# ActiveIntelligentSystemsLab/moving_object_detector

Measured on AMD Instinct MI355X. Metric: stereo pairs/sec (scene-flow+cluster) at 1280x720, higher is better.
Workload: dtype f32+f64; 1 GPU; 1280x720 synthetic sequence (zed-style camera), scene-flow + cluster kernels only (disparity/flow precomputed, HBM-resident), reference default parameters; distinct_frames_per_gpu=16, outputs=six cloud planes, dynamic mask, objects, cluster-label plane, batch_chunks=0, stream=one synthetic stream, contiguous chunk per rank + one disparity plane of halo, collective_executed=True, collective_backend=nccl, collective_on_device=True, collective_world_size=1

## Files before the change

moving_object_detector_amd/csrc/ccl_bits.hip:

```cpp
#include "cluster_common.h"
#pragma clang fp contract(off)
namespace {

namespace bits {
constexpr int TH = 16;

struct Row3 { uint32_t h, a, b; };

__device__ __forceinline__ Row3 operator|(Row3 x, Row3 y) { return {x.h | y.h, x.a | y.a, x.b | y.b}; }
__device__ __forceinline__ Row3 operator&(Row3 x, Row3 y) { return {x.h & y.h, x.a & y.a, x.b & y.b}; }
__device__ __forceinline__ Row3 operator^(Row3 x, Row3 y) { return {x.h ^ y.h, x.a ^ y.a, x.b ^ y.b}; }
__device__ __forceinline__ Row3 andn(Row3 x, Row3 y) { return {x.h & ~y.h, x.a & ~y.a, x.b & ~y.b}; }
__device__ __forceinline__ bool any(Row3 x) { return (x.h | x.a | x.b) != 0u; }
template <int K> __device__ __forceinline__ Row3 shl(Row3 v) {
  return {v.h << K, __builtin_amdgcn_alignbit(v.a, v.h, 32 - K), __builtin_amdgcn_alignbit(v.b, v.a, 32 - K)};
}
template <int K, int NH> __device__ __forceinline__ Row3 shr(Row3 v) {
  return {__builtin_amdgcn_alignbit(v.a, v.h, K) & (~0u << (32 - NH)), __builtin_amdgcn_alignbit(v.b, v.a, K), v.b >> K};
}
__device__ __forceinline__ uint32_t dn1(uint32_t v) { return (uint32_t)__builtin_amdgcn_update_dpp(0, (int)v, 0x138, 0xF, 0xF, false); }
__device__ __forceinline__ uint32_t up1(uint32_t v) { return (uint32_t)__builtin_amdgcn_update_dpp(0, (int)v, 0x130, 0xF, 0xF, false); }
__device__ __forceinline__ Row3 row_dn(Row3 v) { return {dn1(v.h), dn1(v.a), dn1(v.b)}; }
__device__ __forceinline__ Row3 row_up(Row3 v) { return {up1(v.h), up1(v.a), up1(v.b)}; }
template <int K, bool DN> __device__ __forceinline__ Row3 row_shift(Row3 v) {
// ... 54 lines not shown
  return __builtin_amdgcn_readlane(v, 0) + __builtin_amdgcn_readlane(v, 16);
}
__device__ __forceinline__ uint64_t lane_bits(uint32_t lo, uint32_t hi, int l) {
  return ((uint64_t)(uint32_t)__builtin_amdgcn_readlane((int)hi, l) << 32) | (uint64_t)(uint32_t)__builtin_amdgcn_readlane((int)lo, l);
}

constexpr int kTilesPerBlock = 1, kMaxClasses = 4, kMaxComps = 32;

template <class T> __device__ __forceinline__ T ldo(const void *base, uint32_t byte_off) { return *(const T *)((const char *)base + byte_off); }
template <class T> __device__ __forceinline__ void sto(void *base, uint32_t byte_off, T v) { *(T *)((char *)base + byte_off) = v; }

template <int HL>
__global__ __launch_bounds__(64 * kTilesPerBlock) void k_ccl_bits(DevCam c, ClArgs a, int tiles_x, int tiles_y) {
  constexpr int PH = TH + HL;
  const int lane = threadIdx.x, wv = __builtin_amdgcn_readfirstlane((int)threadIdx.y);
  const int wi = blockIdx.x * kTilesPerBlock + wv, ty = blockIdx.y, f = blockIdx.z;
  if (wi >= tiles_x) return;
  const size_t tix = (size_t)f * tiles_y * tiles_x + (size_t)ty * tiles_x + wi;
  int *hdr = a.tilehdr + tix * 2;
  if (__builtin_amdgcn_readfirstlane(hdr[0]) == 0) return;
  const int x0 = wi * 64, y0 = ty * TH, MW = c.mask_words, W = c.W, H = c.H;
  const size_t N = (size_t)W * H, fN = (size_t)f * N;
  Row3 Mrem;
  {
    const int gy = y0 - HL + lane;
    const bool inrow = lane < PH && gy >= 0 && gy < H;
    const uint64_t *mr = a.mask + ((size_t)f * H + (inrow ? gy : 0)) * MW;
    const uint64_t q0 = mr[wi], qL = mr[max(wi - 1, 0)];
    Mrem.h = (inrow && wi > 0) ? ((uint32_t)(qL >> 32) & (~0u << (32 - HL))) : 0u;
    Mrem.a = inrow ? (uint32_t)q0 : 0u;
    Mrem.b = inrow ? (uint32_t)(q0 >> 32) : 0u;
  }
  const bool il = lane >= HL && lane < PH;
  const float th = c.depth_th, qnan = __uint_as_float(0x7fc00000u);
  const uint32_t oc = 4u * (uint32_t)min(x0 + lane, W - 1);
  uint32_t rootA = 0u, rootB = 0u;
  int nreq = 0, ncomp = 0;
  uint2 *req = a.requests + tix * a.req_cap;
  float hi_prev = 0.0f;
  bool bail = false;
  const float *zplane = a.z + fN;
  __shared__ float zlds[kTilesPerBlock][PH][64];
  float(*zl)[64] = zlds[wv];
  float zh[HL];
  float lo = qnan, hi = qnan;
  bool need_z = true;
  if (a.zrange) {
    const int gy = y0 - HL + lane;
    const bool inrow = lane < PH && gy >= 0 && gy < H;
    const float2 *zr = a.zrange + ((size_t)f * H + (inrow ? gy : 0)) * MW;
    const float2 r0 = zr[wi], rL = zr[max(wi - 1, 0)];
    const bool u0 = (Mrem.a | Mrem.b) != 0u, uL = Mrem.h != 0u;
    lo = zmin(u0 ? r0.x : qnan, uL ? rL.x : qnan); hi = zmax(u0 ? r0.y : qnan, uL ? rL.y : qnan);
    lo = wave_fmin(lo); hi = wave_fmax(hi);
    need_z = hi - lo > th;
  }
  if (need_z) {
    lo = qnan; hi = qnan;
    {
      const int gy = min(max(y0 - HL + lane, 0), H - 1);
      const int hx = max(x0 - HL, 0);
#pragma unroll
      for (int j = 0; j < HL; j++) zh[j] = ldo<float>(zplane, 4u * (uint32_t)(gy * W + min(hx + j, W - 1)));
    }
    uint64_t nanb = 0ull;
    constexpr int HB = (PH + 1) / 2;
// ... 90 lines not shown
    const uint64_t ne = __ballot(any(M));
    const int first = __builtin_ctzll(ne);
    const Row3 starts = andn(C, shl<1>(C));
    const bool ok = !any(M) || (popc3(starts) == 1 && !any(E ^ M) && (lane == first || any(M & above)));
    single = __ballot(!ok) == 0ull && __ballot(any(R)) != 0ull;
  }
  for (;;) {
    const uint64_t rrows = __ballot(any(R));
    if (rrows == 0ull) break;
    Row3 S;
    if (single) S = M;
    else {
      const int sr = __builtin_ctzll(rrows);
      const uint32_t sa = (uint32_t)__builtin_amdgcn_readlane((int)R.a, sr), sb = (uint32_t)__builtin_amdgcn_readlane((int)R.b, sr);
      const uint32_t ba = sa & (0u - sa), bb = sa ? 0u : (sb & (0u - sb));
      S = {0u, lane == sr ? ba : 0u, lane == sr ? bb : 0u};
      for (;;) {
        Row3 rA, rX, lA, lX;
        dil_r<HL>(S, rA, rX);
        dil_l<HL>(S, lA, lX);
        const Row3 reach = M & (rA | lA | vert<HL, true>(rA) | vert<HL, false>(lA));
        const Row3 S2 = (fill_up(C, reach) | rev(fill_up(rC, rev(reach)))) & M;
        const bool grew = any(S2 ^ S);
        S = S2;
        if (__ballot(grew) == 0ull) break;
      }
    }
    const uint64_t irows = __ballot(il && (S.a | S.b) != 0u);
    const int rr = __builtin_ctzll(irows);
    const uint32_t fa = (uint32_t)__builtin_amdgcn_readlane((int)S.a, rr), fb = (uint32_t)__builtin_amdgcn_readlane((int)S.b, rr);
    const int rcol = fa ? __builtin_ctz(fa) : 32 + __builtin_ctz(fb);
    const int rootg = (y0 + rr - HL) * W + x0 + rcol;
    if (lane == rr) { if (rcol < 32) rootA |= 1u << rcol; else rootB |= 1u << (rcol - 32); }
    int *pplane = a.parent + fN;
    uint32_t po = 4u * (uint32_t)(y0 * W + x0 + lane);
    asm volatile("" : "+v"(po));
#pragma unroll
    for (int j = 0; j < TH; j++) {
      const uint64_t bitsj = lane_bits(S.a, S.b, HL + j);
      if (bitsj != 0ull && __builtin_amdgcn_inverse_ballot_w64(bitsj))
        sto<int>(pplane, po + 4u * (uint32_t)(j * W), rootg);
    }
    {
      const int cnt = il ? __popc(S.a) + __popc(S.b) : 0;
      const uint32_t ka = S.a & UL.a, kb = S.b & UL.b;
      uint32_t key = (uint32_t)kKeyNone;
      if (il && (ka | kb)) key = (uint32_t)((y0 + lane - HL) * W + x0 + (ka ? __builtin_ctz(ka) : 32 + __builtin_ctz(kb)));
      const int size = wave_sum_lo32(cnt);
      key = wave_min_u32(key);
      if (lane == 0) { sto<int>(a.rsize + fN, 4u * (uint32_t)rootg, size); sto<int>(a.rkey + fN, 4u * (uint32_t)rootg, (int)key); }
    }
    {
      const Row3 HS = {S.h, lane < HL ? S.a : 0u, lane < HL ? S.b : 0u};
      const Row3 em = andn(HS, shl<1>(HS) | row_dn(HS));
      uint64_t todo = __ballot(any(em));
      while (todo) {
        const int l = __builtin_ctzll(todo);
        todo &= todo - 1ull;
        const uint64_t eb = lane_bits(em.a, em.b, l);
        const uint32_t eh = (uint32_t)__builtin_amdgcn_readlane((int)em.h, l) >> (32 - HL);
        const int hgrow = (y0 - HL + l) * W + x0;
        if (__builtin_amdgcn_inverse_ballot_w64((uint64_t)eh)) {
          const int slot = nreq + __popc(eh & ((1u << lane) - 1u));
          if (MOD_CHECK(a, slot < a.req_cap, 12)) req[slot] = make_uint2((uint32_t)(hgrow - HL + lane), (uint32_t)rootg);
        }
        nreq += __popc(eh);
        if (eb != 0ull && __builtin_amdgcn_inverse_ballot_w64(eb)) {
          const int slot = nreq + __popcll((unsigned long long)(eb & ((1ull << lane) - 1ull)));
          if (MOD_CHECK(a, slot < a.req_cap, 12)) req[slot] = make_uint2((uint32_t)(hgrow + lane), (uint32_t)rootg);
        }
        nreq += __popcll((unsigned long long)eb);
      }
    }
    if (single) break;
    R = andn(R, S);
    if (++ncomp >= kMaxComps && __ballot(any(R)) != 0ull) { bail = true; break; }
  }
  {
    uint64_t todo = __ballot((Za | Zb) != 0u);
    while (todo) {
      const int l = __builtin_ctzll(todo);
      todo &= todo - 1ull;
      if (__builtin_amdgcn_inverse_ballot_w64(lane_bits(Za, Zb, l))) {
        const int p = (y0 + l - HL) * W + x0 + lane;
        sto<int>(a.parent + fN, 4u * (uint32_t)p, p); sto<int>(a.rsize + fN, 4u * (uint32_t)p, 1); sto<int>(a.rkey + fN, 4u * (uint32_t)p, kKeyNone);
      }
    }
  }
    if (bail || __ballot(any(Mrem)) == 0ull) break;
  }
  if (bail) {
    if (lane == 0) a.tilelist[atomicAdd(&a.counters[4], 1)] = (uint32_t)tix;
    return;
  }
  if (il && y0 + lane - HL < H) a.lroot[((size_t)f * H + (y0 + lane - HL)) * MW + wi] = ((uint64_t)rootB << 32) | rootA;
  if (lane == 0) { hdr[1] = nreq; hdr[0] = 2; }
}
}
}

void launch_ccl_bits(const DevCam &c, const ClArgs &a, int frames, hipStream_t s) {
  const dim3 tgrid = tile_grid(c, frames);
  const int tx = (int)tgrid.x, tyn = (int)tgrid.y;
  const dim3 bgrid((tgrid.x + bits::kTilesPerBlock - 1) / bits::kTilesPerBlock, tgrid.y, tgrid.z), bblock(64, bits::kTilesPerBlock, 1);
  switch (c.n) {
#define MOD_BITS_CASE(n) case n: hipLaunchKernelGGL(bits::k_ccl_bits<n>, bgrid, bblock, 0, s, c, a, tx, tyn); break;
    MOD_BITS_CASE(1) MOD_BITS_CASE(2) MOD_BITS_CASE(3) MOD_BITS_CASE(4) MOD_BITS_CASE(5)
    MOD_BITS_CASE(6) MOD_BITS_CASE(7) MOD_BITS_CASE(8) MOD_BITS_CASE(9) MOD_BITS_CASE(10)
#undef MOD_BITS_CASE
  }
}
```

moving_object_detector_amd/csrc/ccl_merge.hip:

```cpp
#include "cluster_common.h"
#pragma clang fp contract(off)
namespace {

template <int TH>
__global__ __launch_bounds__(256) void k_tile_flags(DevCam c, ClArgs a, int tiles_x, int tiles_per_frame, int total) {
  const int t = blockIdx.x * 256 + threadIdx.x;
  if (t >= total) return;
  const int f = t / tiles_per_frame, tt = t - f * tiles_per_frame, ty = tt / tiles_x, wi = tt - ty * tiles_x;
  const uint64_t *m = a.mask + ((size_t)f * c.H + (size_t)ty * TH) * c.mask_words + wi;
  const int rows = min(TH, c.H - ty * TH);
  uint64_t any = 0;
#pragma unroll 4
  for (int r = 0; r < rows; r++) any |= m[(size_t)r * c.mask_words];
  a.tilehdr[(size_t)t * 2] = any != 0 ? 1 : 0;
  a.tilehdr[(size_t)t * 2 + 1] = 0;
}

constexpr int kLinkTiles = 32;

__global__ __launch_bounds__(256) void k_ccl_link(DevCam c, ClArgs a, int tiles_per_frame) {
  const int f = blockIdx.y, tid = threadIdx.x, lane = tid & 63;
  const int t0 = blockIdx.x * kLinkTiles;
  int cnt[kLinkTiles], total = 0;
#pragma unroll
  for (int u = 0; u < kLinkTiles; u++) {
    cnt[u] = 0;
    if (t0 + u < tiles_per_frame) {
      const int *hdr = a.tilehdr + ((size_t)f * tiles_per_frame + t0 + u) * 2;
      cnt[u] = hdr[0] ? hdr[1] : 0;
    }
    total += cnt[u];
  }
  if (total == 0) return;
  const size_t N = (size_t)c.W * c.H;
  int *parent = a.parent + (size_t)f * N;
  for (int i0 = 0; i0 < total; i0 += 256) {
    int i = i0 + tid, u = 0;
#pragma unroll
    for (int v = 0; v < kLinkTiles - 1; v++) if (u == v && i >= cnt[v]) { i -= cnt[v]; u = v + 1; }
    int ra = -1, rb = -1;
    if (i0 + tid < total) {
      const uint2 q = a.requests[((size_t)f * tiles_per_frame + t0 + u) * a.req_cap + i];
      if (MOD_CHECK(a, (size_t)q.x < N && (size_t)q.y < N, 0)) { ra = parent[q.x]; rb = (int)q.y; }
      if (!MOD_CHECK(a, ra < 0 || ((size_t)ra < N && rb >= 0), 1)) ra = -1;
    }
    const int pa = wave_prev_i32(ra), pb = wave_prev_i32(rb);
    if (ra >= 0 && !(lane > 0 && pa == ra && pb == rb)) uf_unite(parent, ra, rb);
  }
}

__device__ void select_frame(const DevCam &c, const ClArgs &a, ClusterInfo *tmp, int f, int tid);

template <int TH, bool FILTER>
__global__ __launch_bounds__(256) void k_ccl_merge(DevCam c, ClArgs a, int tiles_per_frame, ClusterInfo *tmp) {
  static_assert(64 % TH == 0, "a wave covers whole tiles");
  constexpr int TPW = 64 / TH;
  const int f = blockIdx.y, lane = threadIdx.x & 63, wv = threadIdx.x >> 6;
  const int t = (blockIdx.x * 4 + wv) * TPW + lane / TH, j = lane % TH;
  const size_t N = (size_t)c.W * c.H;
  int *parent = a.parent + (size_t)f * N;
  int *rsize = a.rsize + (size_t)f * N, *rkey = a.rkey + (size_t)f * N;
  const int wi = t % c.mask_words, ty = t / c.mask_words, y = ty * TH + j;
  unsigned long long bits = 0ull;
  if (t < tiles_per_frame && y < c.H && a.tilehdr[((size_t)f * tiles_per_frame + t) * 2] != 0)
    bits = a.lroot[((size_t)f * c.H + y) * c.mask_words + wi];
  while (bits) {
    const int b = __ffsll(bits) - 1;
    bits &= bits - 1ull;
    const int p = y * c.W + wi * 64 + b;
    const int r = uf_find(parent, p);
    if (!MOD_CHECK(a, r >= 0 && (size_t)r < N, 2)) continue;
    if (r == p) {
      const int slot = atomicAdd(&a.counters[f * 8 + 0], 1);
      if (MOD_CHECK(a, slot >= 0 && (size_t)slot < N, 3)) st_agent(&a.rootlist[(size_t)f * N + slot], p);
    } else {
      parent[p] = r;
// ... 96 lines not shown
```

moving_object_detector_amd/csrc/ccl_tile.hip:

```cpp
#include "cluster_common.h"
#include <algorithm>
#pragma clang fp contract(off)
namespace {

__device__ __forceinline__ void wave_accumulate(int *sizes, int *keys, int stride, int rec_idx, uint32_t key, int lane) {
  uint64_t todo = __ballot(rec_idx >= 0);
  while (todo) {
    const int leader = __ffsll((unsigned long long)todo) - 1;
    const int lid = __builtin_amdgcn_readlane(rec_idx, leader);
    const bool mine = rec_idx == lid;
    const uint64_t grp = __ballot(mine);
    const uint32_t k = wave_min_u32(mine ? key : (uint32_t)kKeyNone);
    if (lane == leader) {
      atomicAdd(&sizes[(size_t)lid * stride], __popcll((unsigned long long)grp));
      if (k != (uint32_t)kKeyNone) atomicMin(&keys[(size_t)lid * stride], (int)k);
    }
    todo &= ~grp;
  }
}

constexpr int kHaloBit = 0x8000;
__device__ __forceinline__ int lds_find(int *L, int a) {
  int p = ld_relaxed(L + (a & 0x7fff));
  while (p != a) {
// ... 292 lines not shown
      float zq[NMAX + 1];
#pragma unroll
      for (int k = 0; k <= NMAX; k++) zq[k] = zt[base - k];
      uint32_t gmask = 0;
#pragma unroll
      for (int k = 0; k <= NMAX; k++) gmask |= (fabsf(zp - zq[k]) > th) ? 0u : (1u << k);
      const uint32_t vmask = cand & gmask;
      const bool need_any = (vmask & dmask) != 0;
      up = up || (vmask != 0);
      if (!MOD_ABLATE(c, 1) && __ballot(need_any)) {
        COUNT(10, 1)
#pragma unroll
        for (int k = 0; k <= NMAX; k++) {
          if (k > n || (dv == 0 && k == 0)) continue;
          const int lab = lq[k];
          const bool need = ((vmask >> k) & 1u) && lab != cur && lab != last;
          if (__ballot(need)) {
            COUNT(12, 1)
            const int pl = wave_prev_i32(lab), pc = wave_prev_i32(cur), pn = wave_prev_i32((int)need);
            push_jobs(need && !(lane > 0 && pn && pc == cur && pl == lab), cur, lab);
            if (need) last = lab;
          }
        }
      }
    }
    STAMP(3)
    upr[j] = up;
  }
  run_jobs();
  lds_barrier();
  STAMP(4)
  int rootg[RPW], rootc[RPW];
  uint64_t rootbits[RPW];
#pragma unroll
  for (int j = 0; j < RPW; j++) {
    const int rr = w + NW * j, gy = y0 + rr;
    const bool dyn = (m0[rr + NMAX] >> lane) & 1ull;
    int rg = -1, rc = -1;
    bool isroot = false;
    if (dyn) {
      const int me = (rr + NMAX) * PW + NMAX + lane;
      const int r = lds_find(Lt, me);
      const int rgr = r / PW, rgc = r - rgr * PW;
      rg = (y0 + rgr - NMAX) * c.W + x0 + rgc - NMAX;
      rc = r;
      if (MOD_CHECK(a, rg >= 0 && (size_t)rg < N && rgr >= NMAX && rgc >= NMAX, 13)) a.parent[fN + (size_t)gy * c.W + x0 + lane] = rg;
      isroot = (r == me);
    }
    rootg[j] = rg; rootc[j] = rc;
    const uint64_t rb = __ballot(isroot);
    rootbits[j] = rb;
    if (lane == 0 && gy < c.H) a.lroot[((size_t)f * c.H + gy) * MW + wi] = rb;
  }
  STAMP(5)
  if (MOD_ABLATE(c, 1 << 18)) return;
  {
    const int topcells = n * (64 + n);
    const int total = topcells + TH * n;
    auto cell_of = [&](int i, int &gr, int &gc) {
      if (i < topcells) { gr = NMAX - n + i / (64 + n); gc = NMAX - n + i % (64 + n); }
      else { const int t = i - topcells; gr = NMAX + t / n; gc = NMAX - n + t % n; }
    };
    auto halo_dyn = [&](int gr, int gc) {
      const int gx = x0 - NMAX + gc;
      const uint64_t mw = (gc >= NMAX) ? m0[gr] : mL[gr];
      return gx >= 0 && ((mw >> (gx & 63)) & 1ull);
    };
    const bool any_halo = !MOD_ABLATE(c, 1024) && s_anyhalo;
    for (int i0 = 0; i0 < total && any_halo; i0 += NW * 64) {
      const int i = i0 + tid;
      if (i < total) {
        int gr, gc;
        cell_of(i, gr, gc);
        if (halo_dyn(gr, gc)) { const int cell = gr * PW + gc; Lt[cell] = lds_find(Lt, cell | kHaloBit); }
      }
    }
    lds_barrier();
    uint2 *req = a.requests + ((size_t)f * tiles_y * tiles_x + (size_t)ty * tiles_x + wi) * a.req_cap;
    for (int i0 = 0; i0 < total && any_halo; i0 += NW * 64) {
      const int i = i0 + tid;
      bool linked = false;
// ... 119 lines not shown
```

moving_object_detector_amd/csrc/cluster_common.h:

```cpp
#pragma once
#include "mod_launch.h"

constexpr int kKeyNone = 0x7fffffff;

__device__ __forceinline__ void lds_barrier() { asm volatile("s_waitcnt lgkmcnt(0)\n\ts_barrier" ::: "memory"); }

__device__ __forceinline__ int ld_relaxed(const int *p) {
  return __hip_atomic_load(p, __ATOMIC_RELAXED, __HIP_MEMORY_SCOPE_WORKGROUP);
}

__device__ __forceinline__ void st_agent(int *p, int v) { __hip_atomic_store(p, v, __ATOMIC_RELAXED, __HIP_MEMORY_SCOPE_AGENT); }
__device__ __forceinline__ int ld_agent(const int *p) { return __hip_atomic_load(p, __ATOMIC_RELAXED, __HIP_MEMORY_SCOPE_AGENT); }

__device__ __forceinline__ int uf_find(const int *parent, int a) {
  int p = ld_relaxed(parent + a);
  while (p != a) { a = p; p = ld_relaxed(parent + a); }
  return a;
}

__device__ __forceinline__ int uf_unite(int *parent, int a, int b) {
  while (true) {
    a = uf_find(parent, a);
    b = uf_find(parent, b);
    if (a == b) return a;
    if (a < b) { const int t = a; a = b; b = t; }
    const int old = atomicMin(&parent[a], b);
    if (old == a) return b;
    a = old;
  }
}

constexpr int kTileH = 16, kTileWaves = 4;
static inline dim3 tile_grid(const DevCam &c, int frames) { return dim3(c.mask_words, ccl_tiles(1, c.H), frames); }
void launch_ccl_bits(const DevCam &c, const ClArgs &a, int frames, hipStream_t s);

#ifdef MOD_PHASE_COUNTERS
#define PHASE_CLOCK unsigned long long pt0 = wall_clock64(), pt1;
#define PHASE_STAMP(i) { __syncthreads(); pt1 = wall_clock64(); if (tid == 0) atomicAdd(&a.dbg[i], pt1 - pt0); pt0 = pt1; }
#else
#define PHASE_CLOCK
#define PHASE_STAMP(i)
#endif


__device__ __forceinline__ uint32_t tie_row_col(uint32_t p, uint32_t W, uint32_t &x) {
  const uint32_t y = p / W;
  x = p - y * W;
  return y;
}

template <int NT> __device__ __forceinline__ void layout_sync() {
  if constexpr (NT == 64) asm volatile("s_waitcnt lgkmcnt(0)" ::: "memory");
  else __syncthreads();
}

struct MemberBox { int xmin, ymin, ymax, ncols; };

template <int NT> __device__ __forceinline__ MemberBox member_box(const uint32_t *pix, int size, uint32_t W, int *s_box, int tid) {
  const int lane = tid & 63;
  if constexpr (NT != 64) {
    if (tid == 0) { s_box[0] = 0x7fffffff; s_box[1] = 0; s_box[2] = 0x7fffffff; s_box[3] = 0; }
    __syncthreads();
  }
  uint32_t x0 = 0xffffffffu, x1 = 0, y0 = 0xffffffffu, y1 = 0;
  for (int i0 = tid; i0 < size; i0 += NT * 4) {
// ... 98 lines not shown
```

moving_object_detector_amd/csrc/cluster_final.hip:

```cpp
#include "cluster_common.h"
#include <algorithm>
#pragma clang fp contract(off)
namespace {

#ifndef FINAL_PLAIN_LABELS
#define FINAL_ST(p, v) __builtin_nontemporal_store((int)(v), (p))
#else
#define FINAL_ST(p, v) (*(p) = (v))
#endif
constexpr int kFinalEarly = 32;
template <int TH, int NW, bool XY_FROM_Z>
__global__ __launch_bounds__(NW * 64) void k_final(DevCam c, ClArgs a) {
  constexpr int RPW = TH / NW;
  __shared__ int nlmap[TH * 64];
  __shared__ int lcount[TH * 64];
  const int wi = blockIdx.x, f = blockIdx.z, lane = threadIdx.x, w = __builtin_amdgcn_readfirstlane((int)threadIdx.y);
  const size_t tidx = (size_t)f * gridDim.y * gridDim.x + (size_t)blockIdx.y * gridDim.x + wi;
  const size_t N = (size_t)c.W * c.H;
  const size_t fN = (size_t)f * N;
  const int x0 = wi * 64, y0 = blockIdx.y * TH, r0 = w * RPW, x = x0 + lane;
  if (a.tilehdr[tidx * 2] == 0) {
    if (a.labels) {
#pragma unroll
      for (int j = 0; j < RPW; j++) { const int y = y0 + r0 + j; if (y < c.H && x < c.W) FINAL_ST(&a.labels[fN + (size_t)y * c.W + x], -1); }
    }
    return;
  }
  const int xc = min(x, c.W - 1);
  uint64_t mw[RPW], rw[RPW];
  int par[RPW];
#pragma unroll
  for (int j = 0; j < RPW; j++) {
    const int y = y0 + r0 + j, yc = min(y, c.H - 1);
    const size_t wo = ((size_t)f * c.H + yc) * c.mask_words + wi;
    mw[j] = (y < c.H) ? a.mask[wo] : 0ull;
    rw[j] = (y < c.H) ? a.lroot[wo] : 0ull;
    par[j] = a.parent[fN + (size_t)yc * c.W + xc];
  }
#pragma unroll
  for (int j = 0; j < RPW; j++) {
    if ((rw[j] >> lane) & 1ull) {
      const int cell = (r0 + j) * 64 + lane;
      const int p = (y0 + r0 + j) * c.W + x;
      int lab = -1, first = 0;
      if (MOD_CHECK(a, par[j] >= 0 && (size_t)par[j] < N, 5)) {
        const int fr = par[j];
        lab = a.rkey[fN + fr];
        const int seg = a.rsize[fN + fr];
        const int own = a.rkey[fN + p];
        first = seg + (fr == p ? 0 : own);
      }
      nlmap[cell] = lab;
      lcount[cell] = first;
    }
  }
  float vx[RPW], vy[RPW], vz[RPW], px[RPW], py[RPW], pz[RPW];
  int ndyn = 0;
#pragma unroll
  for (int j = 0; j < RPW; j++) ndyn += __popcll((unsigned long long)mw[j]);
  const bool early = ndyn >= kFinalEarly;
  auto load_members = [&]() {
#pragma unroll
    for (int j = 0; j < RPW; j++) {
      const size_t gp = fN + (size_t)min(y0 + r0 + j, c.H - 1) * c.W + xc;
      vx[j] = a.vx[gp]; vy[j] = a.vy[gp]; vz[j] = a.vz[gp];
      pz[j] = a.z[gp];
      if (!XY_FROM_Z) { px[j] = a.x[gp]; py[j] = a.y[gp]; }
    }
  };
  if (early) load_members();
  lds_barrier();
  if (w == 0 && lane == 0) a.tilehdr[tidx * 2] = 0;
  const float invW = 1.0f / (float)c.W;
  const int tile0 = y0 * c.W + x0;
  int nl[RPW], cell[RPW], slot[RPW];
  bool any_member = false;
#pragma unroll
  for (int j = 0; j < RPW; j++) {
    const int y = y0 + r0 + j;
    const bool dyn = (mw[j] >> lane) & 1ull;
    const int d = par[j] - tile0;
    const int ly = (int)(((float)d + 0.5f) * invW);
    const bool isroot = (rw[j] >> lane) & 1ull;
    int cl = !dyn ? 0 : isroot ? ((r0 + j) * 64 + lane) : (ly * 64 + (d - ly * c.W));
    if (!MOD_CHECK(a, cl >= 0 && cl < TH * 64 && (!dyn || isroot || (d >= 0 && d - ly * c.W < 64)), 6)) cl = 0;
    int l = dyn ? nlmap[cl] : -1;
    if (!MOD_CHECK(a, l >= -1 && l < a.max_objects, 7)) l = -1;
    nl[j] = l; cell[j] = cl; slot[j] = 0;
    if (a.labels && y < c.H && x < c.W) FINAL_ST(&a.labels[fN + (size_t)y * c.W + x], l);
    any_member = any_member || (__ballot(l >= 0) != 0);
  }
  if (any_member) {
    if (!early) load_members();
#pragma unroll
    for (int j = 0; j < RPW; j++) {
      const int l = nl[j], cl = cell[j];
      const uint64_t mb = __ballot(l >= 0);
      if (mb == 0) continue;
      const int lead = __ffsll((unsigned long long)mb) - 1;
      const int c0 = __builtin_amdgcn_readlane(cl, lead);
      const bool grp = l >= 0 && cl == c0;
      const uint64_t gb = __ballot(grp);
      int base = 0;
      if (lane == lead) base = atomicAdd(&lcount[c0], __popcll((unsigned long long)gb));
      base = __builtin_amdgcn_readlane(base, lead);
      if (grp) slot[j] = base + __popcll((unsigned long long)(gb & ((1ull << lane) - 1ull)));
      else if (l >= 0) slot[j] = atomicAdd(&lcount[cl], 1);
    }
    if (XY_FROM_Z) {
      const double rx = c.rayx[xc];
#pragma unroll
      for (int j = 0; j < RPW; j++) {
        const double zd = (double)pz[j];
        px[j] = (float)(rx * zd);
        py[j] = (float)(c.rayy[min(y0 + r0 + j, c.H - 1)] * zd);
      }
    }
    uint32_t nb[RPW];
// ... 128 lines not shown
```

moving_object_detector_amd/csrc/mod_context.h:

```cpp
#pragma once
#include "../../include/mod_sf.h"
#include "frame_const.h"
#include "mod_launch.h"

#include <string>
#include <utility>
#include <vector>

constexpr int kRing = 4;
constexpr int kMaxChunks = 4;

template <class H, auto Release>
class Owned {
  H h_ = nullptr;

 public:
  Owned() = default;
  Owned(Owned &&o) noexcept : h_(std::exchange(o.h_, nullptr)) {}
  Owned &operator=(Owned &&o) noexcept { std::swap(h_, o.h_); return *this; }
  ~Owned() { reset(); }
  operator H() const { return h_; }
  H get() const { return h_; }
  H *put() { reset(); return &h_; }
  void reset() { if (h_) (void)Release(h_); h_ = nullptr; }
};
template <class T> using DevPtr = Owned<T *, hipFree>;
template <class T> using HostPtr = Owned<T *, hipHostFree>;
using Event = Owned<hipEvent_t, hipEventDestroy>;
using Stream = Owned<hipStream_t, hipStreamDestroy>;

template <class T>
hipError_t dalloc(DevPtr<T> &p, size_t count) { return p ? hipSuccess : hipMalloc((void **)p.put(), count * sizeof(T)); }
inline hipError_t make_event(Event &e) { return e ? hipSuccess : hipEventCreateWithFlags(e.put(), hipEventDisableTiming); }
#define HIP_OK(expr) do { if (hipError_t e_ = (expr); e_ != hipSuccess) return e_; } while (0)

struct Fence {
  Event ev;
  bool armed = false;
  hipError_t record(hipStream_t s) {
    hipError_t e = make_event(ev);
    if (e == hipSuccess && (e = hipEventRecord(ev, s)) == hipSuccess) armed = true;
    return e;
  }
  hipError_t wait(hipStream_t s) const { return armed ? hipStreamWaitEvent(s, ev, 0) : hipSuccess; }
  hipError_t wait_once(hipStream_t s) { return std::exchange(armed, false) ? hipStreamWaitEvent(s, ev, 0) : hipSuccess; }
};

struct EventPair { Event a, b; };

struct ClusterScratch {
  size_t frames = 0, pixels = 0, mask_rows = 0, tiles = 0, max_objects = 0;
  DevPtr<uint64_t> mask, lroot;
  DevPtr<float2> zrange;
  DevPtr<int32_t> parent, rsize, rkey;
  DevPtr<uint32_t> mbits, mpix;
  DevPtr<ClusterBox> cbox;
  DevPtr<ClusterInfo> clusters;
  DevPtr<uint32_t> worklist;
  ClusterInfo *rank_scratch = nullptr; uint32_t *tielist = nullptr;
  DevPtr<int32_t> counters, tilehdr;
  DevPtr<uint32_t> tilelist;
  DevPtr<uint2> requests; size_t req_alloc = 0;
};

struct Buffers {
  DevPtr<double> rayx, rayy;
  DevPtr<FrameConst> fc;
  DevPtr<unsigned long long> dbg;
  ClusterScratch cluster;
  struct Sgm {
    DevPtr<uint32_t> census;
    DevPtr<uint8_t> maps;
    DevPtr<uint8_t> S;
    int D = 0, G = 0; bool maps16 = false;
    Stream side[kSgmPaths];
    Event fork[2], join[2][kSgmPaths];
    DevPtr<float> unfilled; int unfilled_frames = 0;
  } sgm;
  struct Speckle { DevPtr<int32_t> parent, size; int frames = 0; } spk;
  struct Flow {
    DevPtr<uint8_t> img;
    DevPtr<uint32_t> census;
    DevPtr<short2> winners;
    DevPtr<short4> sub;
    DevPtr<float2> unfiltered;
    DevPtr<float2> unfilled;
  } flow;
// ... 246 lines not shown
```

moving_object_detector_amd/csrc/mod_launch.h:

```cpp
#pragma once
#include "../../include/mod_sf.h"
#include "mod_device.h"
#include "label_palette.h"
#include "depth_rays.h"

struct SfArgs {
  const float *dnow, *dprev, *flow;
  float *x, *y, *z, *vx, *vy, *vz;
  uint64_t *mask;
  float4 *aos;
  float *depth;
  float *sflow;
  const FrameConst *fc;
  int32_t *tilehdr;
  int32_t tile_rows, tiles_x, tiles_per_frame;
  float2 *zrange;
  unsigned long long *dbg;
};

constexpr int kClusterCounters = 8;
constexpr int kTileHdrWords = 2;

struct ClArgs {
  const float *x, *y, *z, *vx, *vy, *vz;
  const uint64_t *mask;
  const float2 *zrange;
  uint64_t *lroot;
  int32_t *parent;
  int32_t *rootlist;
  int32_t *labels;
  int32_t *rsize;
  int32_t *rkey;
  ClusterBox *cbox;
  int32_t *counters;
  ClusterInfo *clusters;
  uint32_t *mbits;
  uint32_t *mpix;
  uint32_t *worklist;
  uint32_t *tielist;
  void *objects;
  int32_t *n_objects;
  int32_t *n_clusters;
  int32_t max_objects;
  int32_t xy_from_z;
  uint2 *requests;
  int32_t *tilehdr;
  uint32_t *tilelist;
  int32_t req_cap;
  unsigned long long *dbg;
};

#define MOD_SF_INLINE_FRAMES 8
void launch_scene_flow(const DevCam &c, const SfArgs &a, int frames, const FrameConst *inline_consts, hipStream_t s);
void launch_dynamic_mask(const DevCam &c, int frames, const float *vx, const float *vy, const float *vz, uint64_t *mask,
                         hipStream_t s);
void launch_depth(const DevCam &c, int frames, const float *dnow, float *depth, hipStream_t s);
void launch_copy_words(const unsigned long long *src, unsigned long long *dst, size_t n, hipStream_t s);
void launch_pack(size_t n, const float *x, const float *y, const float *z, const float *vx, const float *vy, const float *vz,
                 void *aos, hipStream_t s);
void launch_unpack(size_t n, const void *aos, float *x, float *y, float *z, float *vx, float *vy, float *vz, hipStream_t s);

// ... 123 lines not shown
```

moving_object_detector_amd/csrc/mod_sf.hip:

```cpp
#include "mod_context.h"
#include "exact_div.h"
#include "flow_color.h"
#include "mod_sf_debug.h"

#include <algorithm>
#include <cmath>
#include <cstdlib>
#include <cstring>
#include <limits>
#include <string>

namespace {

constexpr int kChunkMinFrames = 32;
constexpr int kAutoChunks = 1;

float ceil_to_f32(double th) {
  if (std::isnan(th)) return std::nanf("");
  float t = (float)th;
  if ((double)t < th) t = std::nextafterf(t, INFINITY);
  return t;
}
float floor_to_f32(double th) {
  if (std::isnan(th)) return std::nanf("");
// ... 54 lines not shown
  const int slot = c->ring_pos;
  c->ring_pos = (c->ring_pos + 1) % kRing;
  HIP_TRY(c, hipEventSynchronize(c->pinned_ev[slot]));
  FrameConst *h = c->pinned[slot];
  for (int f = 0; f < in->frames; f++) fill_frame_const(h[f], in->transforms[f], in->dt[f]);
  launch_copy_words((const unsigned long long *)h, (unsigned long long *)c->b.fc.get(), sizeof(FrameConst) / 8 * (size_t)in->frames, c->stream);
  HIP_TRY(c, hipGetLastError());
  HIP_TRY(c, hipEventRecord(c->pinned_ev[slot], c->stream));
  return MOD_OK;
}

int check_batch(ModContext *c, const ModFrameBatch *in) {
  if (!in) return fail(c, MOD_ERR_INVALID_ARGUMENT, "null batch");
  int rc = check_ready(c, in->frames);
  if (rc) return rc;
  return construct_skip(in->flow, in->disparity_prev, in->transforms && in->dt, in->disparity_now);
}

struct Chunk { int f0, n; };

template <class T> T *at(T *p, size_t f0, size_t stride) { return p ? p + f0 * stride : nullptr; }

hipError_t cluster_alloc(ClusterScratch &s, const ModConfig &cfg, int max_objects) {
  s.frames = (size_t)cfg.max_frames; s.pixels = (size_t)cfg.max_width * cfg.max_height; s.max_objects = (size_t)max_objects;
  s.mask_rows = (size_t)mod_mask_words(cfg.max_width) * cfg.max_height; s.tiles = (size_t)ccl_tiles(mod_mask_words(cfg.max_width), cfg.max_height);
  const size_t F = s.frames, FN = F * s.pixels, FM = F * s.mask_rows, FO = F * s.max_objects, FT = F * s.tiles;
  HIP_OK(dalloc(s.mask, FM)); HIP_OK(dalloc(s.lroot, FM)); HIP_OK(dalloc(s.zrange, FM));
  HIP_OK(dalloc(s.parent, FN)); HIP_OK(dalloc(s.rsize, FN)); HIP_OK(dalloc(s.rkey, FN));
  HIP_OK(dalloc(s.cbox, FO)); HIP_OK(dalloc(s.counters, F * kClusterCounters));
  HIP_OK(dalloc(s.clusters, 2 * FO)); s.rank_scratch = s.clusters + FO;
  HIP_OK(dalloc(s.mbits, FN)); HIP_OK(dalloc(s.mpix, FN));
  HIP_OK(dalloc(s.worklist, 2 * FO)); s.tielist = s.worklist + FO;
  HIP_OK(dalloc(s.tilehdr, FT * kTileHdrWords));
  return dalloc(s.tilelist, FT);
}

hipError_t cluster_grow_requests(ClusterScratch &s, int n, hipStream_t stream) {
  const size_t need = s.frames * s.tiles * ccl_request_capacity(n);
  if (need <= s.req_alloc) return hipSuccess;
  HIP_OK(hipStreamSynchronize(stream));
  s.requests.reset(); s.req_alloc = 0;
  HIP_OK(dalloc(s.requests, need));
  s.req_alloc = need; return hipSuccess;
}

struct Carved { ClArgs a; ClusterInfo *rank_scratch; float2 *zrange; int tiles; ClusterMemberOut members; };

Carved cluster_carve(const Buffers &b, const DevCam &dc, Chunk ch, const ModSceneFlowPlanes *pl, const uint64_t *mask, bool flags_ready, const ModClusterOut *out,
                     const ModClusterMembers *mem) {
  const ClusterScratch &s = b.cluster;
  const size_t N = (size_t)dc.W * dc.H, f0 = (size_t)ch.f0, MWH = (size_t)dc.mask_words * dc.H, MO = s.max_objects, tiles = (size_t)ccl_tiles(dc.mask_words, dc.H);
  static const ModClusterOut no_out{}; if (!out) out = &no_out;
  Carved v{{}, s.rank_scratch + f0 * MO, s.zrange + f0 * MWH, (int)tiles, {}}; ClArgs &a = v.a;
  if (mem) v.members = {at(mem->offsets, f0, MO + 1), at(mem->indices, f0, N), at(mem->points, f0, 3 * N)};
  a.x = at(pl->x, f0, N); a.y = at(pl->y, f0, N); a.z = at(pl->z, f0, N); a.vx = at(pl->vx, f0, N); a.vy = at(pl->vy, f0, N); a.vz = at(pl->vz, f0, N);
  a.mask = at(mask, f0, MWH); a.zrange = flags_ready ? v.zrange : nullptr; a.lroot = s.lroot + f0 * MWH;
  a.parent = s.parent + f0 * N; a.rootlist = (int32_t *)s.mpix.get() + f0 * N; a.rsize = s.rsize + f0 * N; a.rkey = s.rkey + f0 * N;
  a.cbox = s.cbox + f0 * MO; a.counters = s.counters + f0 * kClusterCounters; a.clusters = s.clusters + f0 * MO;
  a.mbits = s.mbits + f0 * N; a.mpix = s.mpix + f0 * N; a.worklist = s.worklist + f0 * MO; a.tielist = s.tielist + f0 * MO;
  a.labels = at(out->labels, f0, N); a.objects = at(out->objects, f0, MO); a.n_objects = at(out->n_objects, f0, 1); a.n_clusters = at(out->n_clusters, f0, 1);
  a.max_objects = (int32_t)MO; a.req_cap = ccl_request_capacity(dc.n); a.dbg = b.dbg; a.xy_from_z = flags_ready ? 1 : 0;
  a.requests = s.requests + f0 * tiles * (size_t)a.req_cap; a.tilehdr = s.tilehdr + f0 * tiles * kTileHdrWords; a.tilelist = s.tilelist + f0 * tiles;
  return v;
}

int check_scene_flow_out(ModContext *c, const ModSceneFlowPlanes *out, bool xy_optional) {
  if (!out || !out->z || !out->vx || !out->vy || !out->vz)
    return fail(c, MOD_ERR_INVALID_ARGUMENT, "scene-flow output planes z,vx,vy,vz are required");
  if ((out->x == nullptr) != (out->y == nullptr) || (!out->x && !xy_optional))
    return fail(c, MOD_ERR_INVALID_ARGUMENT, xy_optional ? "scene-flow output planes x and y: pass both or neither" : "scene-flow output planes x,y,z,vx,vy,vz are required");
  return MOD_OK;
}

void enqueue_scene_flow(ModContext *c, const ModFrameBatch *in, const ModSceneFlowPlanes *out, uint64_t *mask, bool tile_flags, Chunk ch,
                        hipStream_t s, const InlineConsts *inl = nullptr) {
  const size_t N = (size_t)c->dc.W * c->dc.H, f0 = (size_t)ch.f0;
  const bool marks = tile_flags && mask;
  const Carved cv = cluster_carve(c->b, c->dc, ch, out, mask, marks, nullptr, nullptr);
  SfArgs a;
  a.dnow = in->disparity_now + f0 * N; a.dprev = in->disparity_prev + f0 * N; a.flow = in->flow + f0 * N * 2;
  a.x = at(out->x, f0, N); a.y = at(out->y, f0, N); a.z = out->z + f0 * N; a.vx = out->vx + f0 * N; a.vy = out->vy + f0 * N; a.vz = out->vz + f0 * N;
  a.mask = at(mask, f0, (size_t)c->dc.mask_words * c->dc.H);
  a.aos = at((float4 *)out->cloud_aos, f0, N * 2); a.depth = at(out->depth, f0, N); a.sflow = at(out->static_flow, f0, N * 2);
  a.fc = c->b.fc + f0; a.dbg = c->b.dbg;
  a.tilehdr = marks ? cv.a.tilehdr : nullptr;
  a.zrange = marks ? cv.zrange : nullptr;
  a.tile_rows = ccl_tile_rows(); a.tiles_x = c->dc.mask_words; a.tiles_per_frame = cv.tiles;
  StageTimer t(c, MOD_STAGE_SCENE_FLOW, s);
  launch_scene_flow(c->dc, a, ch.n, (inl && inl->used) ? inl->v : nullptr, s);
}

int run_scene_flow(ModContext *c, const ModFrameBatch *in, const ModSceneFlowPlanes *out, uint64_t *mask, bool tile_flags, bool xy_optional) {
  int rc = check_scene_flow_out(c, out, xy_optional);
  if (rc) return rc;
  InlineConsts inl;
// ... 533 lines not shown
```

Measured before the change: 99520 stereo pairs/s.

## Store per-pixel tile-local parent as 16-bit cells instead of global int parent

Tile-level CCL kernels now record each dynamic pixel's root as a 16-bit tile-local cell index in a new per-tile tparent buffer. The full 32-bit global parent is written only for root pixels. Merge and final kernels read the compact cell and rebuild global indices, which drops the float-division parent decoding and most parent/rkey loads. This reduces scattered 32-bit parent stores and loads, at the cost of an extra buffer, index reconstruction in merge, and writes for every row that holds any dynamic pixel.

```diff
diff --git a/moving_object_detector_amd/csrc/ccl_bits.hip b/moving_object_detector_amd/csrc/ccl_bits.hip
--- a/moving_object_detector_amd/csrc/ccl_bits.hip
+++ b/moving_object_detector_amd/csrc/ccl_bits.hip
@@ -110,6 +110,10 @@
     Mrem.b = inrow ? (uint32_t)(q0 >> 32) : 0u;
   }
   const bool il = lane >= HL && lane < PH;
+  const uint64_t dynrows = __ballot(il && (Mrem.a | Mrem.b) != 0u) >> HL;
+  uint32_t tp[TH / 2];
+#pragma unroll
+  for (int k = 0; k < TH / 2; k++) tp[k] = 0xFFFFFFFFu;
   const float th = c.depth_th, qnan = __uint_as_float(0x7fc00000u);
   const uint32_t oc = 4u * (uint32_t)min(x0 + lane, W - 1);
   uint32_t rootA = 0u, rootB = 0u;
@@ -266,14 +270,14 @@
     const int rcol = fa ? __builtin_ctz(fa) : 32 + __builtin_ctz(fb);
     const int rootg = (y0 + rr - HL) * W + x0 + rcol;
     if (lane == rr) { if (rcol < 32) rootA |= 1u << rcol; else rootB |= 1u << (rcol - 32); }
-    int *pplane = a.parent + fN;
-    uint32_t po = 4u * (uint32_t)(y0 * W + x0 + lane);
-    asm volatile("" : "+v"(po));
-#pragma unroll
-    for (int j = 0; j < TH; j++) {
-      const uint64_t bitsj = lane_bits(S.a, S.b, HL + j);
-      if (bitsj != 0ull && __builtin_amdgcn_inverse_ballot_w64(bitsj))
-        sto<int>(pplane, po + 4u * (uint32_t)(j * W), rootg);
+    {
+      const uint32_t rc2 = (uint32_t)((rr - HL) * 64 + rcol) * 0x10001u;
+#pragma unroll
+      for (int k = 0; k < TH / 2; k++) {
+        const uint32_t m = (__builtin_amdgcn_inverse_ballot_w64(lane_bits(S.a, S.b, HL + 2 * k)) ? 0x0000FFFFu : 0u) |
+                           (__builtin_amdgcn_inverse_ballot_w64(lane_bits(S.a, S.b, HL + 2 * k + 1)) ? 0xFFFF0000u : 0u);
+        tp[k] = (tp[k] & ~m) | (rc2 & m);
+      }
     }
     {
       const int cnt = il ? __popc(S.a) + __popc(S.b) : 0;
@@ -282,7 +286,9 @@
       if (il && (ka | kb)) key = (uint32_t)((y0 + lane - HL) * W + x0 + (ka ? __builtin_ctz(ka) : 32 + __builtin_ctz(kb)));
       const int size = wave_sum_lo32(cnt);
       key = wave_min_u32(key);
-      if (lane == 0) { sto<int>(a.rsize + fN, 4u * (uint32_t)rootg, size); sto<int>(a.rkey + fN, 4u * (uint32_t)rootg, (int)key); }
+      if (lane == 0) {
+        sto<int>(a.parent + fN, 4u * (uint32_t)rootg, rootg); sto<int>(a.rsize + fN, 4u * (uint32_t)rootg, size); sto<int>(a.rkey + fN, 4u * (uint32_t)rootg, (int)key);
+      }
     }
     {
       const Row3 HS = {S.h, lane < HL ? S.a : 0u, lane < HL ? S.b : 0u};
@@ -312,6 +318,14 @@
   }
   {
     uint64_t todo = __ballot((Za | Zb) != 0u);
+    if (todo) {
+#pragma unroll
+      for (int k = 0; k < TH / 2; k++) {
+        const uint32_t m = (__builtin_amdgcn_inverse_ballot_w64(lane_bits(Za, Zb, HL + 2 * k)) ? 0x0000FFFFu : 0u) |
+                           (__builtin_amdgcn_inverse_ballot_w64(lane_bits(Za, Zb, HL + 2 * k + 1)) ? 0xFFFF0000u : 0u);
+        tp[k] = (tp[k] & ~m) | ((uint32_t)((2 * k * 64 + lane) | ((2 * k * 64 + 64 + lane) << 16)) & m);
+      }
+    }
     while (todo) {
       const int l = __builtin_ctzll(todo);
       todo &= todo - 1ull;
@@ -326,6 +340,14 @@
   if (bail) {
     if (lane == 0) a.tilelist[atomicAdd(&a.counters[4], 1)] = (uint32_t)tix;
     return;
+  }
+  {
+    uint16_t *tpt = a.tparent + tix * (size_t)kTileParentCells;
+#pragma unroll
+    for (int k = 0; k < TH / 2; k++) {
+      if ((dynrows >> (2 * k)) & 1ull) sto<uint16_t>(tpt, 2u * (uint32_t)(2 * k * 64 + lane), (uint16_t)tp[k]);
+      if ((dynrows >> (2 * k + 1)) & 1ull) sto<uint16_t>(tpt, 2u * (uint32_t)(2 * k * 64 + 64 + lane), (uint16_t)(tp[k] >> 16));
+    }
   }
   if (il && y0 + lane - HL < H) a.lroot[((size_t)f * H + (y0 + lane - HL)) * MW + wi] = ((uint64_t)rootB << 32) | rootA;
   if (lane == 0) { hdr[1] = nreq; hdr[0] = 2; }
diff --git a/moving_object_detector_amd/csrc/ccl_merge.hip b/moving_object_detector_amd/csrc/ccl_merge.hip
--- a/moving_object_detector_amd/csrc/ccl_merge.hip
+++ b/moving_object_detector_amd/csrc/ccl_merge.hip
@@ -41,7 +41,12 @@
     int ra = -1, rb = -1;
     if (i0 + tid < total) {
       const uint2 q = a.requests[((size_t)f * tiles_per_frame + t0 + u) * a.req_cap + i];
-      if (MOD_CHECK(a, (size_t)q.x < N && (size_t)q.y < N, 0)) { ra = parent[q.x]; rb = (int)q.y; }
+      if (MOD_CHECK(a, (size_t)q.x < N && (size_t)q.y < N, 0)) {
+        const int hy = (int)(q.x / (uint32_t)c.W), hx = (int)q.x - hy * c.W;
+        const int hty = hy / kTileH, hwi = hx >> 6;
+        const uint32_t cell = a.tparent[((size_t)f * tiles_per_frame + (size_t)hty * c.mask_words + hwi) * kTileParentCells + (hy - hty * kTileH) * 64 + (hx & 63)];
+        if (MOD_CHECK(a, cell < (uint32_t)kTileParentCells, 1)) { ra = (hty * kTileH + (int)(cell >> 6)) * c.W + hwi * 64 + (int)(cell & 63u); rb = (int)q.y; }
+      }
       if (!MOD_CHECK(a, ra < 0 || ((size_t)ra < N && rb >= 0), 1)) ra = -1;
     }
     const int pa = wave_prev_i32(ra), pb = wave_prev_i32(rb);
diff --git a/moving_object_detector_amd/csrc/ccl_tile.hip b/moving_object_detector_amd/csrc/ccl_tile.hip
--- a/moving_object_detector_amd/csrc/ccl_tile.hip
+++ b/moving_object_detector_amd/csrc/ccl_tile.hip
@@ -348,11 +348,14 @@
   STAMP(4)
   int rootg[RPW], rootc[RPW];
   uint64_t rootbits[RPW];
+  uint16_t *tpt = a.tparent + ((size_t)f * tiles_y * tiles_x + (size_t)ty * tiles_x + wi) * (size_t)kTileParentCells;
 #pragma unroll
   for (int j = 0; j < RPW; j++) {
     const int rr = w + NW * j, gy = y0 + rr;
-    const bool dyn = (m0[rr + NMAX] >> lane) & 1ull;
+    const uint64_t mrow = m0[rr + NMAX];
+    const bool dyn = (mrow >> lane) & 1ull;
     int rg = -1, rc = -1;
+    uint32_t tcell = 0xFFFFu;
     bool isroot = false;
     if (dyn) {
       const int me = (rr + NMAX) * PW + NMAX + lane;
@@ -360,9 +363,13 @@
       const int rgr = r / PW, rgc = r - rgr * PW;
       rg = (y0 + rgr - NMAX) * c.W + x0 + rgc - NMAX;
       rc = r;
-      if (MOD_CHECK(a, rg >= 0 && (size_t)rg < N && rgr >= NMAX && rgc >= NMAX, 13)) a.parent[fN + (size_t)gy * c.W + x0 + lane] = rg;
       isroot = (r == me);
-    }
+      if (MOD_CHECK(a, rg >= 0 && (size_t)rg < N && rgr >= NMAX && rgc >= NMAX, 13)) {
+        tcell = (uint32_t)((rgr - NMAX) * 64 + (rgc - NMAX));
+        if (isroot) a.parent[fN + (size_t)rg] = rg;
+      }
+    }
+    if (mrow != 0ull) tpt[(uint32_t)(rr * 64 + lane)] = (uint16_t)tcell;
     rootg[j] = rg; rootc[j] = rc;
     const uint64_t rb = __ballot(isroot);
     rootbits[j] = rb;
diff --git a/moving_object_detector_amd/csrc/cluster_common.h b/moving_object_detector_amd/csrc/cluster_common.h
--- a/moving_object_detector_amd/csrc/cluster_common.h
+++ b/moving_object_detector_amd/csrc/cluster_common.h
@@ -31,6 +31,7 @@
 }
 
 constexpr int kTileH = 16, kTileWaves = 4;
+static_assert(kTileParentCells == kTileH * 64, "ClArgs.tparent holds one 16-bit cell per pixel of a tile");
 static inline dim3 tile_grid(const DevCam &c, int frames) { return dim3(c.mask_words, ccl_tiles(1, c.H), frames); }
 void launch_ccl_bits(const DevCam &c, const ClArgs &a, int frames, hipStream_t s);
 
diff --git a/moving_object_detector_amd/csrc/cluster_final.hip b/moving_object_detector_amd/csrc/cluster_final.hip
--- a/moving_object_detector_amd/csrc/cluster_final.hip
+++ b/moving_object_detector_amd/csrc/cluster_final.hip
@@ -19,7 +19,16 @@
   const size_t N = (size_t)c.W * c.H;
   const size_t fN = (size_t)f * N;
   const int x0 = wi * 64, y0 = blockIdx.y * TH, r0 = w * RPW, x = x0 + lane;
-  if (a.tilehdr[tidx * 2] == 0) {
+  const int hdr0 = a.tilehdr[tidx * 2];
+  uint64_t rw[RPW];
+  {
+    const char *lr = (const char *)(a.lroot + (size_t)f * c.H * c.mask_words + wi);
+#pragma unroll
+    for (int j = 0; j < RPW; j++) rw[j] = *(const uint64_t *)(lr + 8u * (uint32_t)(min(y0 + r0 + j, c.H - 1) * c.mask_words));
+  }
+#pragma unroll
+  for (int j = 0; j < RPW; j++) asm volatile("" : "+s"(rw[j]));
+  if (hdr0 == 0) {
     if (a.labels) {
 #pragma unroll
       for (int j = 0; j < RPW; j++) { const int y = y0 + r0 + j; if (y < c.H && x < c.W) FINAL_ST(&a.labels[fN + (size_t)y * c.W + x], -1); }
@@ -27,15 +36,18 @@
     return;
   }
   const int xc = min(x, c.W - 1);
-  uint64_t mw[RPW], rw[RPW];
-  int par[RPW];
+  uint64_t mw[RPW];
+  int par[RPW], own[RPW];
+  uint32_t tcell[RPW];
+  const uint16_t *tpt = a.tparent + tidx * (size_t)kTileParentCells;
 #pragma unroll
   for (int j = 0; j < RPW; j++) {
     const int y = y0 + r0 + j, yc = min(y, c.H - 1);
-    const size_t wo = ((size_t)f * c.H + yc) * c.mask_words + wi;
-    mw[j] = (y < c.H) ? a.mask[wo] : 0ull;
-    rw[j] = (y < c.H) ? a.lroot[wo] : 0ull;
-    par[j] = a.parent[fN + (size_t)yc * c.W + xc];
+    mw[j] = (y < c.H) ? a.mask[((size_t)f * c.H + yc) * c.mask_words + wi] : 0ull;
+    if (y >= c.H) rw[j] = 0ull;
+    tcell[j] = tpt[(r0 + j) * 64 + lane];
+    par[j] = 0; own[j] = 0;
+    if ((rw[j] >> lane) & 1ull) { const size_t p = fN + (size_t)y * c.W + x; par[j] = a.parent[p]; own[j] = a.rkey[p]; }
   }
 #pragma unroll
   for (int j = 0; j < RPW; j++) {
@@ -47,8 +59,7 @@
         const int fr = par[j];
         lab = a.rkey[fN + fr];
         const int seg = a.rsize[fN + fr];
-        const int own = a.rkey[fN + p];
-        first = seg + (fr == p ? 0 : own);
+        first = seg + (fr == p ? 0 : own[j]);
       }
       nlmap[cell] = lab;
       lcount[cell] = first;
@@ -71,19 +82,14 @@
   if (early) load_members();
   lds_barrier();
   if (w == 0 && lane == 0) a.tilehdr[tidx * 2] = 0;
-  const float invW = 1.0f / (float)c.W;
-  const int tile0 = y0 * c.W + x0;
   int nl[RPW], cell[RPW], slot[RPW];
   bool any_member = false;
 #pragma unroll
   for (int j = 0; j < RPW; j++) {
     const int y = y0 + r0 + j;
     const bool dyn = (mw[j] >> lane) & 1ull;
-    const int d = par[j] - tile0;
-    const int ly = (int)(((float)d + 0.5f) * invW);
-    const bool isroot = (rw[j] >> lane) & 1ull;
-    int cl = !dyn ? 0 : isroot ? ((r0 + j) * 64 + lane) : (ly * 64 + (d - ly * c.W));
-    if (!MOD_CHECK(a, cl >= 0 && cl < TH * 64 && (!dyn || isroot || (d >= 0 && d - ly * c.W < 64)), 6)) cl = 0;
+    int cl = dyn ? (int)tcell[j] : 0;
+    if (!MOD_CHECK(a, cl >= 0 && cl < TH * 64, 6)) cl = 0;
     int l = dyn ? nlmap[cl] : -1;
     if (!MOD_CHECK(a, l >= -1 && l < a.max_objects, 7)) l = -1;
     nl[j] = l; cell[j] = cl; slot[j] = 0;
diff --git a/moving_object_detector_amd/csrc/mod_context.h b/moving_object_detector_amd/csrc/mod_context.h
--- a/moving_object_detector_amd/csrc/mod_context.h
+++ b/moving_object_detector_amd/csrc/mod_context.h
@@ -53,6 +53,7 @@
   DevPtr<uint64_t> mask, lroot;
   DevPtr<float2> zrange;
   DevPtr<int32_t> parent, rsize, rkey;
+  DevPtr<uint16_t> tparent;
   DevPtr<uint32_t> mbits, mpix;
   DevPtr<ClusterBox> cbox;
   DevPtr<ClusterInfo> clusters;
diff --git a/moving_object_detector_amd/csrc/mod_launch.h b/moving_object_detector_amd/csrc/mod_launch.h
--- a/moving_object_detector_amd/csrc/mod_launch.h
+++ b/moving_object_detector_amd/csrc/mod_launch.h
@@ -20,6 +20,7 @@
 
 constexpr int kClusterCounters = 8;
 constexpr int kTileHdrWords = 2;
+constexpr int kTileParentCells = 16 * 64;
 
 struct ClArgs {
   const float *x, *y, *z, *vx, *vy, *vz;
@@ -27,6 +28,7 @@
   const float2 *zrange;
   uint64_t *lroot;
   int32_t *parent;
+  uint16_t *tparent;
   int32_t *rootlist;
   int32_t *labels;
   int32_t *rsize;
diff --git a/moving_object_detector_amd/csrc/mod_sf.hip b/moving_object_detector_amd/csrc/mod_sf.hip
--- a/moving_object_detector_amd/csrc/mod_sf.hip
+++ b/moving_object_detector_amd/csrc/mod_sf.hip
@@ -110,6 +110,7 @@
   HIP_OK(dalloc(s.mbits, FN)); HIP_OK(dalloc(s.mpix, FN));
   HIP_OK(dalloc(s.worklist, 2 * FO)); s.tielist = s.worklist + FO;
   HIP_OK(dalloc(s.tilehdr, FT * kTileHdrWords));
+  HIP_OK(dalloc(s.tparent, FT * kTileParentCells));
   return dalloc(s.tilelist, FT);
 }
 
@@ -139,6 +140,7 @@
   a.labels = at(out->labels, f0, N); a.objects = at(out->objects, f0, MO); a.n_objects = at(out->n_objects, f0, 1); a.n_clusters = at(out->n_clusters, f0, 1);
   a.max_objects = (int32_t)MO; a.req_cap = ccl_request_capacity(dc.n); a.dbg = b.dbg; a.xy_from_z = flags_ready ? 1 : 0;
   a.requests = s.requests + f0 * tiles * (size_t)a.req_cap; a.tilehdr = s.tilehdr + f0 * tiles * kTileHdrWords; a.tilelist = s.tilelist + f0 * tiles;
+  a.tparent = s.tparent + f0 * tiles * kTileParentCells;
   return v;
 }
 
```

Result: no change. 99410 stereo pairs/s (-0.1%).
